# LGMOak/HighPerformanceComputing-LatticeBoltzmannMethod

Hardware: AMD Instinct MI355X
Metric: MLUPS (fp64) (higher is better)
Workload: dtype f64

## Files before the change

highperformancecomputing-latticeboltzmannmethod_amd/csrc/lbm_kernel_col.hpp:

```cpp
#pragma once
#include "lbm_kernels.hpp"

namespace lbmk {

__device__ __forceinline__ unsigned dpp_shr1(unsigned v) { return (unsigned)__builtin_amdgcn_mov_dpp((int)v, 0x138, 0xf, 0xf, true); }
__device__ __forceinline__ unsigned dpp_shl1(unsigned v) { return (unsigned)__builtin_amdgcn_mov_dpp((int)v, 0x130, 0xf, 0xf, true); }
__device__ __forceinline__ double from_left(double v) {
    const unsigned long long u = __builtin_bit_cast(unsigned long long, v);
    const unsigned lo = dpp_shr1((unsigned)u), hi = dpp_shr1((unsigned)(u >> 32));
    return __builtin_bit_cast(double, ((unsigned long long)hi << 32) | lo);
}
__device__ __forceinline__ double from_right(double v) {
    const unsigned long long u = __builtin_bit_cast(unsigned long long, v);
    const unsigned lo = dpp_shl1((unsigned)u), hi = dpp_shl1((unsigned)(u >> 32));
    return __builtin_bit_cast(double, ((unsigned long long)hi << 32) | lo);
}
__device__ __forceinline__ float from_left(float v) { return __builtin_bit_cast(float, dpp_shr1(__builtin_bit_cast(unsigned, v))); }
__device__ __forceinline__ float from_right(float v) { return __builtin_bit_cast(float, dpp_shl1(__builtin_bit_cast(unsigned, v))); }

template <int NW> constexpr int col_waves_per_simd() { return NW == 12 ? 6 : NW <= 8 ? (2 * NW) / 4 : NW / 4; }
template <typename T, int NW, int AR> constexpr int col_min_waves() {
    return (sizeof(T) == 4 && NW == 8 && AR == AR_CONTRACTED_TRT) ? 6 : col_waves_per_simd<NW>();
}

template <typename T, int R, int NW, int D, bool NT, int AR = AR_STRICT>
__global__ void __launch_bounds__(NW * 64, (col_min_waves<T, NW, AR>())) k_stepc_col(const KArgs<T> a, const K2Extra<T> e) {
    constexpr int H = R * NW, HW = D - 1, OW = 64 - 2 * HW, OH = H - 2 * HW, LW = 64 + 2;
    static_assert(D >= 2 && OH >= 1 && R >= 2, "(D <= GR on a strip: its ghost rows go GR deep — the host's business)");
    __shared__ T xbuf[2][NW][6][LW];
    const int lane = (int)threadIdx.x & 63;
    const int w = __builtin_amdgcn_readfirstlane((int)threadIdx.x >> 6);
    const int nbx = (a.nx + OW - 1) / OW, nby = (a.y_cnt + OH - 1) / OH + (a.y_cnt2 + OH - 1) / OH, nb = nbx * nby;
    int b = blockIdx.x;
    { const int per = (int)gridDim.x >> 3; b = (b & 7) * per + (b >> 3); }
    if (b >= nb) return;
    int by = b / nbx;
    const int bx = b - by * nbx;
    if (a.reverse) by = nby - 1 - by;
    int y_end;
    const int Yo = band_origin(a, by, OH, y_end);
    const int Xo = bx * OW;
    const int X0 = Xo - HW, Yr = Yo - HW;
    const int ry0 = w * R;
    const TileFrame<T> fr(a, e, Xo, Yo, y_end, OW, OH, HW);
    const int x = X0 + lane;
    auto run = [&]<bool LEAN>() {
        T g[R][Q];
        bool bad = false;
        const bool col_in = (x >= 0 && x < a.nx);
        unsigned sbits = 0;
        if (!LEAN && fr.near_solid && col_in) {
#pragma unroll
            for (int j = 0; j < R; ++j) {
                const int yg = a.y_start + Yr + ry0 + j;
                if (yg >= 0 && yg < a.ny_glob && solid_at(a, x, yg)) sbits |= 1u << j;
            }
        }
        LBM_PROF_IDS(b, NW, w);
        LBM_PROF(b, NW, w, 0);
        if (LEAN) {
            const unsigned ub = fr.src_off(a, Yr + ry0, X0), voff = (unsigned)lane * (unsigned)sizeof(T);
            auto load_all = [&]<int AUX>() {
#pragma unroll
                for (int j = 0; j < R; ++j) fr.template load<AUX>(g[j], voff, ub + (unsigned)j * fr.pitchB);
            };
            if (e.ntl) load_all.template operator()<2>(); else load_all.template operator()<0>();
#pragma unroll
            for (int j = 0; j < R; ++j) {
                bad |= any_unstable(g[j]);
                collide<T, AR>(g[j], a);
            }
        } else {
#pragma unroll
            for (int j = 0; j < R; ++j) {
                const int y = Yr + ry0 + j, yg = a.y_start + y;
                const bool row_in = (yg >= 0 && yg < a.ny_glob);
                if (!(row_in && col_in) || y > y_end + HW - 1) {
#pragma unroll
                    for (int i = 0; i < Q; ++i) g[j][i] = outside_value(e, row_in, col_in, i);
                } else {
                    const long c = (long)(y + GR) * a.pitch + a.xoff + x;
#pragma unroll
                    for (int i = 0; i < Q; ++i) g[j][i] = a.src[(long)i * a.plane + c - (long)cy(i) * a.pitch - cx(i)];
                    cell_update_as<T, AR, true>(a, g[j], x, yg, 0, (sbits >> j) & 1u, fr.near_solid, true, bad);
                }
            }
        }
        if (bad) atomicMin(a.unstable_t, *a.t_base + a.t);
        LBM_PROF(b, NW, w, 1);
        auto level = [&]<int L>() {
            T (*xb)[6][LW] = xbuf[L & 1];
            const int wb = w > 0 ? w - 1 : 0, wa = w + 1 < NW ? w + 1 : NW - 1;
            xb[w][0][1 + lane] = g[R - 1][2]; xb[w][1][1 + lane] = g[R - 1][5]; xb[w][2][1 + lane] = g[R - 1][6];
            xb[w][3][1 + lane] = g[0][4];     xb[w][4][1 + lane] = g[0][7];     xb[w][5][1 + lane] = g[0][8];
            __syncthreads();
            T p2 = xb[wb][0][1 + lane], p5 = xb[wb][1][lane], p6 = xb[wb][2][2 + lane];
            bool badl = false;
            const bool lane_ok = lane >= L - 1 && lane <= 64 - L;
#pragma unroll
            for (int j = 0; j < R; ++j) {
                const int ry = ry0 + j;
                const T n2 = g[j][2], n5 = g[j][5], n6 = g[j][6];
                if (ry >= L - 1 && ry <= H - L) {
                T f[Q];
                f[0] = g[j][0]; f[1] = from_left(g[j][1]); f[3] = from_right(g[j][3]);
                f[2] = p2; f[5] = p5; f[6] = p6;
                if (j < R - 1) { f[4] = g[j + 1][4]; f[7] = from_right(g[j + 1][7]); f[8] = from_left(g[j + 1][8]); }
                else { f[4] = xb[wa][3][1 + lane]; f[7] = xb[wa][4][2 + lane]; f[8] = xb[wa][5][lane]; }
                const bool valid = lane_ok;
                const int y = Yr + ry, yg = a.y_start + y;
                bool store = L == D && lane >= HW && lane < 64 - HW && ry >= HW && ry < H - HW;
                if (LEAN) {
                    badl |= unstable_if(f, valid);
                    collide<T, AR>(f, a);
                } else {
                    const bool row_in = (yg >= 0 && yg < a.ny_glob);
                    if (!(row_in && col_in)) {
#pragma unroll
                        for (int i = 0; i < Q; ++i) f[i] = outside_value(e, row_in, col_in, i);
                        store = false;
                    } else {
                        cell_update_as<T, AR, true>(a, f, x, yg, L - 1, (sbits >> j) & 1u, fr.near_solid, valid && y <= y_end + HW - L, badl);
                        store = store && y < y_end && !((sbits >> j) & 1u);
                    }
                }
                if (L < D) {
#pragma unroll
                    for (int i = 0; i < Q; ++i) g[j][i] = f[i];
                } else if (store) {
                    if (LEAN) fr.template store<NT>(f, (unsigned)lane * (unsigned)sizeof(T), fr.dst_off(a, y, X0));
                    else store_cell<NT>(a, f, x, y);
                }
                }
                if (j < R - 1) { p2 = n2; p5 = from_left(n5); p6 = from_right(n6); }
            }
            if (badl) atomicMin(a.unstable_t, *a.t_base + a.t + L - 1);
            LBM_PROF(b, NW, w, L);
        };
        [&]<int... Ls>(std::integer_sequence<int, Ls...>) { (level.template operator()<Ls + 2>(), ...); }(std::make_integer_sequence<int, D - 1>{});
    };
    if (fr.lean) run.template operator()<true>();
    else run.template operator()<false>();
}

}
```

highperformancecomputing-latticeboltzmannmethod_amd/csrc/lbm_kernels.hpp:

```cpp
#pragma once
#include <utility>
#include <hip/hip_runtime.h>

namespace lbmk {

constexpr int Q = 9;
constexpr int GR = 12;
constexpr int HR1 = 6;
__host__ __device__ constexpr int cx(int i) { constexpr int v[Q] = {0, 1, 0, -1, 0, 1, -1, -1, 1}; return v[i]; }
__host__ __device__ constexpr int cy(int i) { constexpr int v[Q] = {0, 0, 1, 0, -1, 1, 1, -1, -1}; return v[i]; }
__host__ __device__ constexpr int opp(int i) { constexpr int v[Q] = {0, 3, 4, 1, 2, 7, 8, 5, 6}; return v[i]; }
template <typename T> __host__ __device__ constexpr T wgt(int i) {
    return i == 0 ? T(4.0 / 9.0) : (i < 5 ? T(1.0 / 9.0) : T(1.0 / 36.0));
}

struct MaskView {
    const unsigned long long* bits = nullptr;
    const int* sat = nullptr;
    int y0 = 0, rows = 0, words = 0, nbx = 0, nby = 0;
};
__host__ __device__ inline bool mask_cell(const MaskView& m, int x, int yg) {
    const int r = yg - m.y0;
    if (r < 0 || r >= m.rows) return false;
    return (m.bits[(long)r * m.words + (x >> 6)] >> (x & 63)) & 1ull;
}
__host__ __device__ inline bool mask_box_any(const MaskView& m, int x0, int x1, int yg0, int yg1) {
    x0 = x0 < 0 ? 0 : x0;
    x1 = x1 > m.nbx * 8 - 1 ? m.nbx * 8 - 1 : x1;
    const int r0 = yg0 - m.y0 < 0 ? 0 : yg0 - m.y0, r1 = yg1 - m.y0 > m.rows - 1 ? m.rows - 1 : yg1 - m.y0;
    if (x0 > x1 || r0 > r1) return false;
    const int W = m.nbx + 1, c0 = x0 >> 3, c1 = (x1 >> 3) + 1, b0 = r0 >> 3, b1 = (r1 >> 3) + 1;
    return m.sat[b1 * W + c1] - m.sat[b0 * W + c1] - m.sat[b1 * W + c0] + m.sat[b0 * W + c0] > 0;
}

enum WallKind { WALL_NOSLIP = 0, WALL_FREESLIP = 1, WALL_MOVING = 2 };
__host__ __device__ constexpr int wall_pack(int south, int north) { return south | (north << 2); }
template <typename T> struct WallK { T s_add, s_sub, n_add, n_sub; };
template <typename T>
inline WallK<T> wall_ks(int south, double u_south, int north, double u_north) {
    WallK<T> k;
    k.s_add = south == WALL_MOVING ? (T)(u_south * (1.0 / 6.0)) : T(-0.0);
    k.s_sub = south == WALL_MOVING ? (T)(u_south * (1.0 / 6.0)) : T(0.0);
    k.n_add = north == WALL_MOVING ? (T)(u_north * (1.0 / 6.0)) : T(-0.0);
    k.n_sub = north == WALL_MOVING ? (T)(u_north * (1.0 / 6.0)) : T(0.0);
    return k;
}


template <typename T>
struct KArgs {
    const T* src;
    T* dst;
    long plane;
    int pitch;
    int xoff;
    int nx, ny_loc;
    int ny_glob;
    int y_start;
    int cyl_x, cyl_y;
    double cyl_r2;
    MaskView mv;
    T tau_inv;
    const T* u_row;
    int* unstable_t;
    int t;
    const int* t_base;
    int y_lo, y_cnt;
    int y_lo2, y_cnt2;
    int reverse;
    union { T les_tau; T trt_wm; };
    union { T les_tau2; T trt_wa; };
    union { T les_c; T trt_wb; };
    int walls;
    WallK<T> wk;
    const int* sched;
};

template <typename T>
__device__ __forceinline__ int row_of_block(const KArgs<T>& a) {
    const int by = (int)blockIdx.y;
    if (by >= a.y_cnt) return a.y_lo2 + (by - a.y_cnt);
    return a.y_lo + (a.reverse ? a.y_cnt - 1 - by : by);
}

template <typename T>
__device__ __forceinline__ int band_origin(const KArgs<T>& a, int by, int TY, int& y_end) {
    const int nb1 = (a.y_cnt + TY - 1) / TY;
    if (by >= nb1) { y_end = a.y_lo2 + a.y_cnt2; return a.y_lo2 + (by - nb1) * TY; }
    y_end = a.y_lo + a.y_cnt;
    return a.y_lo + by * TY;
}

__device__ __forceinline__ bool is_solid_cell(int x, int yg, int cyl_x, int cyl_y, double cyl_r2) {
    const double dx = (double)(x - cyl_x), dy = (double)(yg - cyl_y);
    return dx * dx + dy * dy <= cyl_r2;
}

template <typename A>
__device__ __forceinline__ bool solid_at(const A& a, int x, int yg) {
    return a.mv.bits ? mask_cell(a.mv, x, yg) : is_solid_cell(x, yg, a.cyl_x, a.cyl_y, a.cyl_r2);
}

template <typename T>
__device__ __forceinline__ bool tile_near_solid(const KArgs<T>& a, int X0, int Y0, int TX, int TY, int ring) {
    const int yg0 = a.y_start + Y0;
    if (a.mv.bits) return mask_box_any(a.mv, X0 - ring, X0 + TX - 1 + ring, yg0 - ring, yg0 + TY - 1 + ring);
    const int r = (int)sqrt(a.cyl_r2) + 1;
    return X0 - ring <= a.cyl_x + r && X0 + TX - 1 + ring >= a.cyl_x - r &&
           yg0 - ring <= a.cyl_y + r && yg0 + TY - 1 + ring >= a.cyl_y - r;
}

__host__ __device__ inline int inlet_sched_index(int t, int n, int mode) {
    const unsigned ut = (unsigned)t, un = (unsigned)n;
    return (int)(mode == 1 ? ut % un : (ut < un - 1u ? ut : un - 1u));
}
constexpr int INLET_SCHED_HEAD = 2;
template <typename T>
__device__ __forceinline__ T inlet_sched_at(const int* sched, int t) {
    return reinterpret_cast<const T*>(sched + INLET_SCHED_HEAD)[inlet_sched_index(t, sched[0], sched[1])];
}

template <typename T>
__host__ __device__ __forceinline__ void wall_rule(T (&f)[Q], bool bottom, bool top, int walls, const WallK<T>& k) {
    if (bottom) {
        const bool fs = (walls & 3) == WALL_FREESLIP;
        const T a = fs ? f[8] : f[7], b = fs ? f[7] : f[8];
        f[2] = f[4]; f[5] = a + k.s_add; f[6] = b - k.s_sub;
    }
    if (top) {
        const bool fs = ((walls >> 2) & 3) == WALL_FREESLIP;
        const T a = fs ? f[6] : f[5], b = fs ? f[5] : f[6];
        f[4] = f[2]; f[7] = a - k.n_sub; f[8] = b + k.n_add;
    }
}

template <typename T, typename U>
__device__ __forceinline__ void apply_bcs(T (&f)[Q], bool bottom, bool top, bool inlet, bool outlet, U&& inlet_u,
                                          int walls, const WallK<T>& wk, T& rho_bc, T& u_out) {
    wall_rule(f, bottom, top, walls, wk);
    if (inlet) {
        const T u_in = inlet_u();
        rho_bc = (f[0] + f[2] + f[4] + T(2.0) * (f[3] + f[6] + f[7])) / (T(1.0) - u_in);
        f[1] = f[3] + T(2.0 / 3.0) * rho_bc * u_in;
        f[5] = f[7] - T(0.5) * (f[2] - f[4]) + T(1.0 / 6.0) * rho_bc * u_in;
        f[8] = f[6] + T(0.5) * (f[2] - f[4]) + T(1.0 / 6.0) * rho_bc * u_in;
    }
    if (outlet) {
        const T rho_out = T(1.0);
        u_out = T(-1.0) + (f[0] + f[2] + f[4] + T(2.0) * (f[1] + f[5] + f[8])) / rho_out;
        f[3] = f[1] - T(2.0 / 3.0) * rho_out * u_out;
        f[6] = f[8] - T(0.5) * (f[2] - f[4]) - T(1.0 / 6.0) * rho_out * u_out;
        f[7] = f[5] + T(0.5) * (f[2] - f[4]) - T(1.0 / 6.0) * rho_out * u_out;
    }
}
template <typename T>
__device__ __forceinline__ void bcs_at(const KArgs<T>& a, T (&f)[Q], int x, int yg, int lvl) {
    T rho_bc, u_out;
    apply_bcs(f, yg == 0, yg == a.ny_glob - 1, x == 0, x == a.nx - 1, [&]() {
        T u = a.u_row[yg];
        if (a.sched) u = u * inlet_sched_at<T>(a.sched, *a.t_base + a.t + lvl);
        return u;
    }, a.walls, a.wk, rho_bc, u_out);
}

enum Arith { AR_STRICT = 0, AR_CONTRACTED = 1, AR_STRICT_LES = 2, AR_CONTRACTED_LES = 3, AR_STRICT_TRT = 4, AR_CONTRACTED_TRT = 5 };
constexpr bool ar_contracted(int ar) { return (ar & 1) != 0; }
constexpr bool ar_les(int ar) { return (ar & 2) != 0; }
constexpr bool ar_trt(int ar) { return (ar & 4) != 0; }
constexpr int ar_of(bool contracted, bool les, bool trt = false) { return (contracted ? 1 : 0) | (les ? 2 : 0) | (trt ? 4 : 0); }

__device__ __forceinline__ double fma_t(double a, double b, double c) { return __builtin_fma(a, b, c); }
__device__ __forceinline__ float fma_t(float a, float b, float c) { return __builtin_fmaf(a, b, c); }
__device__ __forceinline__ double recip_t(double d) {
    double r = __builtin_amdgcn_rcp(d);
    r = fma_t(fma_t(-d, r, 1.0), r, r);
    r = fma_t(fma_t(-d, r, 1.0), r, r);
    return r;
}
__device__ __forceinline__ float recip_t(float d) {
    float r = __builtin_amdgcn_rcpf(d);
    return fma_t(fma_t(-d, r, 1.0f), r, r);
}
__device__ __forceinline__ double sqrt_t(double v) { return __builtin_sqrt(v); }
__device__ __forceinline__ float sqrt_t(float v) { return __builtin_sqrtf(v); }
__device__ __forceinline__ double sqrt_c(double v) {
    v = __builtin_fmax(v, 1e-300);
    const double y = __builtin_amdgcn_rsq(v);
    const double s = v * y;
    return fma_t(s, fma_t(-s, 0.5 * y, 0.5), s);
}
__device__ __forceinline__ float sqrt_c(float v) { return __builtin_amdgcn_sqrtf(v); }

typedef unsigned lbm_u32x2 __attribute__((ext_vector_type(2)));
__device__ __forceinline__ __amdgpu_buffer_rsrc_t buf_desc(const void* base) {
    return __builtin_amdgcn_make_buffer_rsrc(const_cast<void*>(base), 0, 0xffffffff, 0x00020000);
}
template <typename T, int AUX = 0> __device__ __forceinline__ T buf_load(__amdgpu_buffer_rsrc_t r, unsigned voff, unsigned soff) {
    if constexpr (sizeof(T) == 8) return __builtin_bit_cast(T, __builtin_amdgcn_raw_buffer_load_b64(r, voff, soff, AUX));
    else return __builtin_bit_cast(T, __builtin_amdgcn_raw_buffer_load_b32(r, voff, soff, AUX));
}
template <bool NT> __device__ __forceinline__ void buf_store(double v, __amdgpu_buffer_rsrc_t r, unsigned voff, unsigned soff) {
    __builtin_amdgcn_raw_buffer_store_b64(__builtin_bit_cast(lbm_u32x2, v), r, voff, soff, NT ? 2 : 0);
}
template <bool NT> __device__ __forceinline__ void buf_store(float v, __amdgpu_buffer_rsrc_t r, unsigned voff, unsigned soff) {
    __builtin_amdgcn_raw_buffer_store_b32(__builtin_bit_cast(unsigned, v), r, voff, soff, NT ? 2 : 0);
}

__device__ __forceinline__ void strict_div2(double& a1, double& a2, double b) {
    double r = __builtin_amdgcn_rcp(b);
    double e = __builtin_fma(-b, r, 1.0);
    r = __builtin_fma(r, e, r);
    e = __builtin_fma(-b, r, 1.0);
    r = __builtin_fma(r, e, r);
    double q = a1 * r;
    a1 = __builtin_fma(__builtin_fma(-b, q, a1), r, q);
    q = a2 * r;
    a2 = __builtin_fma(__builtin_fma(-b, q, a2), r, q);
}
__device__ __forceinline__ void strict_div2(float& a1, float& a2, float b) { a1 /= b; a2 /= b; }
template <int UNUSED = 0>
__global__ void k_debug_strict_div2(const double* a1, const double* a2, const double* b, int n, double* q1, double* q2, double* r1, double* r2) {
    const int k = blockIdx.x * blockDim.x + threadIdx.x;
    if (k >= n) return;
    double x = a1[k], y = a2[k];
    strict_div2(x, y, b[k]);
    q1[k] = x; q2[k] = y;
    r1[k] = a1[k] / b[k]; r2[k] = a2[k] / b[k];
}

template <typename T>
__device__ __forceinline__ T les_tau_inv_strict(const T (&f)[Q], T rho, T ux, T uy, T tau, T tau2, T c) {
    const T sxx = ((((f[1] + f[3]) + f[5]) + f[6]) + f[7]) + f[8];
    const T syy = ((((f[2] + f[4]) + f[5]) + f[6]) + f[7]) + f[8];
    const T sxy = ((f[5] - f[6]) + f[7]) - f[8];
    const T pxx = (sxx - rho * (ux * ux)) - rho * T(1.0 / 3.0);
    const T pyy = (syy - rho * (uy * uy)) - rho * T(1.0 / 3.0);
    const T pxy = sxy - rho * (ux * uy);
    const T qn = sqrt_t((pxx * pxx + pyy * pyy) + T(2.0) * (pxy * pxy));
    const T tau_eff = T(0.5) * (tau + sqrt_t(tau2 + c * (qn / rho)));
    return T(1.0) / tau_eff;
}

template <typename T, int AR = AR_STRICT>
__device__ __forceinline__ void bgk_collide(T (&f)[Q], T tau_inv, T les_tau = T(0), T les_tau2 = T(0), T les_c = T(0)) {
    T rho = T(0), ux = T(0), uy = T(0);
    if constexpr (ar_contracted(AR)) {
        const T a13 = f[1] + f[3], a24 = f[2] + f[4], a57 = f[5] + f[7], a68 = f[6] + f[8];
        const T d13 = f[1] - f[3], d24 = f[2] - f[4], d57 = f[5] - f[7], d68 = f[6] - f[8];
        rho = ((f[0] + a13) + (a24 + a57)) + a68;
        ux = (d13 + d57) - d68;
        uy = (d24 + d57) + d68;
        const T rinv = recip_t(rho);
        const T inv3 = rinv * T(3.0);
        const T vx = ux * inv3, vy = uy * inv3;
        if constexpr (ar_les(AR)) {
            const T sxx = (a13 + a57) + a68, syy = (a24 + a57) + a68, sxy = a57 - a68;
            const T jxr = ux * rinv;
            const T third = rho * T(-1.0 / 3.0);
            const T pxx = fma_t(-jxr, ux, sxx + third), pyy = fma_t(-uy * rinv, uy, syy + third), pxy = fma_t(-jxr, uy, sxy);
            const T qn = sqrt_c(fma_t(pxx, pxx, fma_t(pyy, pyy, T(2.0) * (pxy * pxy))));
            tau_inv = T(2.0) * recip_t(les_tau + sqrt_c(fma_t(les_c, qn * rinv, les_tau2)));
        }
        const T base = fma_t(T(-1.0 / 6.0), fma_t(vx, vx, vy * vy), T(1.0));
        const T wr0 = wgt<T>(0) * rho, wr1 = wgt<T>(1) * rho, wr5 = wgt<T>(5) * rho;
        if constexpr (ar_trt(AR)) {
            const T wa = les_tau2, wb = les_c;
            f[0] = fma_t(tau_inv, fma_t(wr0, base, -f[0]), f[0]);
            auto pair = [&](int i, int ib, T cv, T wr) {
                const T ri = fma_t(wr, fma_t(cv, fma_t(cv, T(0.5), T(1.0)), base), -f[i]);
                const T rb = fma_t(wr, fma_t(cv, fma_t(cv, T(0.5), T(-1.0)), base), -f[ib]);
                f[i] = fma_t(wa, ri, fma_t(wb, rb, f[i]));
                f[ib] = fma_t(wa, rb, fma_t(wb, ri, f[ib]));
            };
            auto then = [&](int i, int ib, int j, int jb) { asm volatile("" : "+v"(f[i]), "+v"(f[ib]), "+v"(f[j]), "+v"(f[jb])); };
            pair(5, 7, vx + vy, wr5);
            then(5, 7, 8, 6);
            pair(8, 6, vx - vy, wr5);
            then(8, 6, 1, 3);
            pair(1, 3, vx, wr1);
            then(1, 3, 2, 4);
            pair(2, 4, vy, wr1);
            return;
        }
#pragma unroll
        for (int i = 0; i < Q; ++i) {
            T cv;
            if (cx(i) == 0 && cy(i) == 0) cv = T(0);
            else if (cy(i) == 0) cv = T(cx(i)) * vx;
            else if (cx(i) == 0) cv = T(cy(i)) * vy;
            else cv = T(cx(i)) * vx + T(cy(i)) * vy;
            const T t = (i == 0) ? base : fma_t(cv, fma_t(cv, T(0.5), T(1.0)), base);
            const T wr = i == 0 ? wr0 : (i < 5 ? wr1 : wr5);
            f[i] = fma_t(tau_inv, fma_t(wr, t, -f[i]), f[i]);
        }
        return;
    }
#pragma unroll
    for (int i = 0; i < Q; ++i) {
        rho += f[i];
        if (cx(i) != 0) ux += T(cx(i)) * f[i];
        if (cy(i) != 0) uy += T(cy(i)) * f[i];
    }
    strict_div2(ux, uy, rho);
    if constexpr (ar_les(AR)) tau_inv = les_tau_inv_strict(f, rho, ux, uy, les_tau, les_tau2, les_c);
    const T usq = ux * ux + uy * uy;
    const T c15 = T(1.5) * usq;
    const T wr0 = wgt<T>(0) * rho, wr1 = wgt<T>(1) * rho, wr5 = wgt<T>(5) * rho;
    auto relax = [&](T& fi, T wr, T bracket) {
        const T feq = wr * bracket;
        fi = fi - tau_inv * (fi - feq);
    };
    relax(f[0], wr0, (T(1.0) + T(0.0)) - c15);
    auto pair = [&](int i, int ib, T cu, T wr) {
        const T t3 = T(3.0) * cu, t45 = (T(4.5) * cu) * cu;
        if constexpr (ar_trt(AR)) {
            const T feq = wr * (((T(1.0) + t3) + t45) - c15), feqb = wr * (((T(1.0) - t3) + t45) - c15);
            const T np = T(0.5) * ((f[i] + f[ib]) - (feq + feqb));
            const T nm = T(0.5) * ((f[i] - f[ib]) - (feq - feqb));
            const T wpn = tau_inv * np, wmn = les_tau * nm;
            f[i] = (f[i] - wpn) - wmn;
            f[ib] = (f[ib] - wpn) + wmn;
            return;
        }
        relax(f[i], wr, ((T(1.0) + t3) + t45) - c15);
        relax(f[ib], wr, ((T(1.0) - t3) + t45) - c15);
    };
    pair(1, 3, ux, wr1);
    pair(2, 4, uy, wr1);
    pair(5, 7, ux + uy, wr5);
    pair(8, 6, ux - uy, wr5);
}

template <typename T, int AR>
__device__ __forceinline__ void collide(T (&f)[Q], const KArgs<T>& a) {
    static_assert(!(ar_les(AR) && ar_trt(AR)), "TRT and LES exclude each other");
    if constexpr (ar_trt(AR)) bgk_collide<T, AR>(f, a.tau_inv, a.trt_wm, a.trt_wa, a.trt_wb);
    else if constexpr (ar_les(AR)) bgk_collide<T, AR>(f, T(0), a.les_tau, a.les_tau2, a.les_c);
    else bgk_collide<T, AR>(f, a.tau_inv);
}

__device__ __forceinline__ unsigned exp_word(double v) { return (unsigned)(__builtin_bit_cast(unsigned long long, v) >> 32); }
__device__ __forceinline__ unsigned exp_word(float v) { return __builtin_bit_cast(unsigned, v); }
template <typename T>
__device__ __forceinline__ bool any_unstable(const T (&f)[Q]) {
    unsigned o = 0;
#pragma unroll
    for (int i = 0; i < Q; ++i) o |= exp_word(f[i]);
    bool bad = false;
    if (o & 0x40000000u) {
#pragma unroll
        for (int i = 0; i < Q; ++i) bad |= !(fabs(f[i]) <= T(1e5));
    }
    return bad;
}
template <typename T>
__device__ __forceinline__ bool unstable_if(const T (&f)[Q], bool valid) {
    unsigned o = 0;
#pragma unroll
    for (int i = 0; i < Q; ++i) o |= exp_word(f[i]);
    o = valid ? o : 0u;
    bool bad = false;
    if (o & 0x40000000u) {
#pragma unroll
        for (int i = 0; i < Q; ++i) bad |= !(fabs(f[i]) <= T(1e5));
        bad = bad && valid;
    }
    return bad;
}

enum StepMode { MODE_STEP = 0, MODE_COLLIDE_ONLY = 1, MODE_STREAM_ONLY = 2 };

template <typename T, int MODE, bool NT = false, int AR = AR_STRICT>
__global__ void __launch_bounds__(256) k_step_site(const KArgs<T> a) {
    const int x = blockIdx.x * 256 + threadIdx.x;
    const int y = row_of_block(a);
    if (x >= a.nx) return;
    const int yg = a.y_start + y;
    const long c = (long)(y + GR) * a.pitch + a.xoff + x;
    T f[Q];
#pragma unroll
    for (int i = 0; i < Q; ++i) {
        const long off = (MODE == MODE_COLLIDE_ONLY) ? 0 : (long)cy(i) * a.pitch + cx(i);
        f[i] = a.src[(long)i * a.plane + c - off];
    }
    const bool solid = solid_at(a, x, yg);
    if (MODE != MODE_COLLIDE_ONLY && !solid) bcs_at(a, f, x, yg, 0);
    if (MODE == MODE_STEP) {
        if (any_unstable(f)) atomicMin(a.unstable_t, *a.t_base + a.t);
    }
    if (MODE == MODE_STREAM_ONLY) {
        if (solid) {
            T r[Q];
#pragma unroll
            for (int i = 0; i < Q; ++i) r[i] = f[opp(i)];
#pragma unroll
            for (int i = 0; i < Q; ++i) f[i] = r[i];
        }
    } else {
        if (solid) return;
        collide<T, AR>(f, a);
    }
#pragma unroll
    for (int i = 0; i < Q; ++i) {
        T* p = a.dst + (long)i * a.plane + c;
        if (NT) __builtin_nontemporal_store(f[i], p);
        else *p = f[i];
    }
}


template <typename T> struct K2Extra {
    const T* feq_in;
    int small;
    int xcd;
    int nt;
    int ntl;
};


template <typename T, int AR, bool BRANCH_FREE = false>
__device__ __forceinline__ void cell_update_as(const KArgs<T>& a, T (&f)[Q], int x, int yg, int lvl, bool solid, bool near_solid,
                                               bool count, bool& bad) {
    if (!solid) bcs_at(a, f, x, yg, lvl);
    if (BRANCH_FREE) bad |= unstable_if(f, count);
    else if (count) bad |= any_unstable(f);
    collide<T, AR>(f, a);
    if (near_solid) {
#pragma unroll
        for (int i = 0; i < Q; ++i) f[i] = solid ? wgt<T>(i) : f[i];
    }
}
template <typename T, int AR>
__device__ __forceinline__ void cell_update(const KArgs<T>& a, T (&f)[Q], int x, int yg, int lvl, bool near_solid, bool count, bool& bad) {
    bool solid = false;
    if (near_solid) solid = solid_at(a, x, yg);
    cell_update_as<T, AR>(a, f, x, yg, lvl, solid, near_solid, count, bad);
}
template <typename T, int AR>
__device__ __forceinline__ bool cell_update_last(const KArgs<T>& a, T (&f)[Q], int x, int yg, int lvl, bool near_solid, bool& bad) {
    const bool solid = near_solid && solid_at(a, x, yg);
    if (!solid) bcs_at(a, f, x, yg, lvl);
    bad |= any_unstable(f);
    if (solid) return false;
    collide<T, AR>(f, a);
    return true;
}

template <typename T>
__device__ __forceinline__ T outside_value(const K2Extra<T>& e, bool row_in, bool col_in, int i) {
    return (row_in && !col_in) ? T(0) : e.feq_in[i];
}
template <bool NT, typename T>
__device__ __forceinline__ void store_cell(const KArgs<T>& a, const T (&f)[Q], int x, int y) {
    T* base = a.dst + ((long)(y + GR) * a.pitch + a.xoff + x);
#pragma unroll
    for (int i = 0; i < Q; ++i) {
        if (NT) __builtin_nontemporal_store(f[i], base + (long)i * a.plane); else base[(long)i * a.plane] = f[i];
    }
}
template <typename T>
__device__ __forceinline__ void store_cell(const KArgs<T>& a, const T (&f)[Q], int x, int y, bool nt) {
    if (nt) store_cell<true>(a, f, x, y); else store_cell<false>(a, f, x, y);
}

template <typename T>
struct TileFrame {
    int X0, Y0;
    int y_end;
    bool near_solid;
    bool lean;
    unsigned pitchB, planeB, KB;
    __amdgpu_buffer_rsrc_t rsrc, rdst;

    __device__ __forceinline__ TileFrame(const KArgs<T>& a, const K2Extra<T>& e, int X0_, int Y0_, int y_end_, int OW, int OH, int HW)
        : X0(X0_), Y0(Y0_), y_end(y_end_) {
        near_solid = tile_near_solid(a, X0, Y0, OW, OH, HW);
        const int yg0 = a.y_start + Y0;
        lean = !near_solid && X0 >= HW + 1 && X0 + OW + HW <= a.nx - 1 && yg0 >= HW + 1 && yg0 + OH + HW <= a.ny_glob - 1 &&
               Y0 + OH <= y_end && e.small;
        pitchB = (unsigned)a.pitch * (unsigned)sizeof(T);
        planeB = (unsigned)a.plane * (unsigned)sizeof(T);
        KB = pitchB + (unsigned)sizeof(T);
        rsrc = buf_desc(reinterpret_cast<const char*>(a.src) - KB);
        rdst = buf_desc(a.dst);
    }
    __device__ __forceinline__ unsigned src_off(const KArgs<T>& a, int y, int x) const {
        return (unsigned)(y + GR) * pitchB + (unsigned)(a.xoff + x) * (unsigned)sizeof(T) + KB;
    }
    __device__ __forceinline__ unsigned dst_off(const KArgs<T>& a, int y, int x) const {
        return (unsigned)(y + GR) * pitchB + (unsigned)(a.xoff + x) * (unsigned)sizeof(T);
    }
    __device__ __forceinline__ unsigned at(int row, int col) const { return (unsigned)row * pitchB + (unsigned)col * (unsigned)sizeof(T); }
    template <int AUX = 0>
    __device__ __forceinline__ void load(T (&f)[Q], unsigned voff, unsigned soff) const {
#pragma unroll
        for (int i = 0; i < Q; ++i)
            f[i] = buf_load<T, AUX>(rsrc, voff, soff + (unsigned)i * planeB - (unsigned)cy(i) * pitchB - (unsigned)(cx(i) * (int)sizeof(T)));
    }
    template <bool NT>
    __device__ __forceinline__ void store(const T (&f)[Q], unsigned voff, unsigned soff) const {
#pragma unroll
        for (int i = 0; i < Q; ++i) buf_store<NT>(f[i], rdst, voff, soff + (unsigned)i * planeB);
    }
    __device__ __forceinline__ void store(const T (&f)[Q], unsigned voff, unsigned soff, bool nt) const {
        if (nt) store<true>(f, voff, soff); else store<false>(f, voff, soff);
    }
};

template <typename T>
__device__ __forceinline__ TileFrame<T> tile_frame(const KArgs<T>& a, const K2Extra<T>& e, int TX, int TY, int HW) {
    int bx = blockIdx.x, by = blockIdx.y;
    if (e.xcd) {
        const int nb = gridDim.x * gridDim.y;
        int b = by * gridDim.x + bx;
        if (nb % 8 == 0) b = (b % 8) * (nb / 8) + b / 8;
        by = b / gridDim.x; bx = b - by * gridDim.x;
    }
    if (a.reverse) by = (int)gridDim.y - 1 - by;
    int y_end;
    const int Y0 = band_origin(a, by, TY, y_end);
    return TileFrame<T>(a, e, bx * TX, Y0, y_end, TX, TY, HW);
}

template <typename T, int TY, int NTH, int AR = AR_STRICT>
__global__ void __launch_bounds__(NTH) k_step2_tile(const KArgs<T> a, const K2Extra<T> e) {
    constexpr int TX = 64, RW = TX + 2, RH = TY + 2, LP = RW + 2;
    __shared__ T lds[Q][RH][LP];
    const TileFrame<T> fr = tile_frame(a, e, TX, TY, 1);
    const int X0 = fr.X0, Y0 = fr.Y0, y_end = fr.y_end;
    bool bad = false;
    for (int r = threadIdx.x; r < RW * RH; r += NTH) {
        const int ry = r / RW, rx = r - ry * RW;
        const int x = X0 + rx - 1, y = Y0 + ry - 1;
        if (y > y_end) continue;
        const int yg = a.y_start + y;
        const bool row_in = (yg >= 0 && yg < a.ny_glob), col_in = (x >= 0 && x < a.nx);
        T f[Q];
        if (!(row_in && col_in)) {
#pragma unroll
            for (int i = 0; i < Q; ++i) f[i] = outside_value(e, row_in, col_in, i);
        } else {
            const long c = (long)(y + GR) * a.pitch + a.xoff + x;
#pragma unroll
            for (int i = 0; i < Q; ++i) f[i] = a.src[(long)i * a.plane + c - (long)cy(i) * a.pitch - cx(i)];
            cell_update<T, AR>(a, f, x, yg, 0, fr.near_solid, true, bad);
        }
#pragma unroll
        for (int i = 0; i < Q; ++i) lds[i][ry][rx] = f[i];
    }
    if (bad) atomicMin(a.unstable_t, *a.t_base + a.t);
    __syncthreads();
    bad = false;
    for (int o = threadIdx.x; o < TX * TY; o += NTH) {
        const int ly = o / TX, lx = o - ly * TX;
        const int x = X0 + lx, y = Y0 + ly;
        if (y >= y_end || x >= a.nx) continue;
        T f[Q];
#pragma unroll
        for (int i = 0; i < Q; ++i) f[i] = lds[i][ly + 1 - cy(i)][lx + 1 - cx(i)];
        if (cell_update_last<T, AR>(a, f, x, a.y_start + y, 1, fr.near_solid, bad)) store_cell(a, f, x, y, e.nt != 0);
    }
    if (bad) atomicMin(a.unstable_t, *a.t_base + a.t + 1);
}

template <typename T, int TY, int NTH, int D, int AR>
__device__ __forceinline__ void step_tile(const KArgs<T>& a, const K2Extra<T>& e) {
    constexpr int TX = 64, HW = D - 1, R1W = TX + 2 * HW, R1H = TY + 2 * HW, LP = R1W;
    static_assert((R1W - 2) * (R1H - 2) <= 2 * NTH, "two cells per thread at most in the in-place levels");
    __shared__ T lds[Q][R1H][LP];
    const TileFrame<T> fr = tile_frame(a, e, TX, TY, HW);
    const int X0 = fr.X0, Y0 = fr.Y0, y_end = fr.y_end;
    auto run = [&]<bool LEAN>() {
        bool bad = false;
#pragma unroll
        for (int r = threadIdx.x; r < R1W * R1H; r += NTH) {
            const int ry = r / R1W, rx = r - ry * R1W;
            T f[Q];
            if (LEAN) {
                fr.load(f, fr.at(ry, rx), fr.src_off(a, Y0 - HW, X0 - HW));
                bad |= any_unstable(f);
                collide<T, AR>(f, a);
            } else {
                const int x = X0 + rx - HW, y = Y0 + ry - HW;
                const int yg = a.y_start + y;
                const bool row_in = (yg >= 0 && yg < a.ny_glob), col_in = (x >= 0 && x < a.nx);
                if (!(row_in && col_in) || y > y_end + HW - 1) {
#pragma unroll
                    for (int i = 0; i < Q; ++i) f[i] = outside_value(e, row_in, col_in, i);
                } else {
                    const long c = (long)(y + GR) * a.pitch + a.xoff + x;
#pragma unroll
                    for (int i = 0; i < Q; ++i) f[i] = a.src[(long)i * a.plane + c - (long)cy(i) * a.pitch - cx(i)];
                    cell_update<T, AR>(a, f, x, yg, 0, fr.near_solid, true, bad);
                }
            }
#pragma unroll
            for (int i = 0; i < Q; ++i) lds[i][ry][rx] = f[i];
        }
        if (bad) atomicMin(a.unstable_t, *a.t_base + a.t);
        __syncthreads();
        auto in_place = [&]<int L>() {
            constexpr int O = L - 1, RW = R1W - 2 * O, RH = R1H - 2 * O;
            T g[2][Q];
            int cell[2];
#pragma unroll
            for (int k = 0; k < 2; ++k) {
                const int r = (int)threadIdx.x + k * NTH;
                cell[k] = (r < RW * RH) ? r : -1;
                if (cell[k] >= 0) {
                    const int ry = r / RW + O, rx = r - (r / RW) * RW + O;
#pragma unroll
                    for (int i = 0; i < Q; ++i) g[k][i] = lds[i][ry - cy(i)][rx - cx(i)];
                }
            }
            __syncthreads();
            bool badl = false;
#pragma unroll
            for (int k = 0; k < 2; ++k) {
                if (cell[k] < 0) continue;
                const int r = cell[k];
                const int ry = r / RW + O, rx = r - (r / RW) * RW + O;
                const int x = X0 + rx - HW, y = Y0 + ry - HW;
                const int yg = a.y_start + y;
                const bool row_in = (yg >= 0 && yg < a.ny_glob), col_in = (x >= 0 && x < a.nx);
                T f[Q];
                if (!LEAN && !(row_in && col_in)) {
#pragma unroll
                    for (int i = 0; i < Q; ++i) f[i] = outside_value(e, row_in, col_in, i);
                } else {
#pragma unroll
                    for (int i = 0; i < Q; ++i) f[i] = g[k][i];
                    if (LEAN) {
                        badl |= any_unstable(f);
                        collide<T, AR>(f, a);
                    } else cell_update<T, AR>(a, f, x, yg, L - 1, fr.near_solid, y <= y_end + HW - L, badl);
                }
#pragma unroll
                for (int i = 0; i < Q; ++i) lds[i][ry][rx] = f[i];
            }
            if (badl) atomicMin(a.unstable_t, *a.t_base + a.t + L - 1);
            __syncthreads();
        };
        [&]<int... Ls>(std::integer_sequence<int, Ls...>) { (in_place.template operator()<Ls + 2>(), ...); }(std::make_integer_sequence<int, D - 2>{});
        bad = false;
        for (int o = threadIdx.x; o < TX * TY; o += NTH) {
            const int ly = o / TX, lx = o - ly * TX;
            const int x = X0 + lx, y = Y0 + ly;
            if (!LEAN && (y >= y_end || x >= a.nx)) continue;
            T f[Q];
#pragma unroll
            for (int i = 0; i < Q; ++i) f[i] = lds[i][ly + HW - cy(i)][lx + HW - cx(i)];
            if (LEAN) {
                bad |= any_unstable(f);
                collide<T, AR>(f, a);
                fr.store(f, fr.at(ly, lx), fr.dst_off(a, Y0, X0), e.nt != 0);
            } else if (cell_update_last<T, AR>(a, f, x, a.y_start + y, D - 1, fr.near_solid, bad)) store_cell(a, f, x, y, e.nt != 0);
        }
        if (bad) atomicMin(a.unstable_t, *a.t_base + a.t + D - 1);
    };
    if (fr.lean) run.template operator()<true>();
    else run.template operator()<false>();
}
template <typename T, int TY, int NTH, int AR = AR_STRICT>
__global__ void __launch_bounds__(NTH, (2 * NTH / 256)) k_step3_tile(const KArgs<T> a, const K2Extra<T> e) { step_tile<T, TY, NTH, 3, AR>(a, e); }
template <typename T, int TY, int NTH, int AR = AR_STRICT>
__global__ void __launch_bounds__(NTH, (2 * NTH / 256)) k_step4_tile(const KArgs<T> a, const K2Extra<T> e) { step_tile<T, TY, NTH, 4, AR>(a, e); }

#ifdef LBM_COL_PROF
constexpr int PROF_SLOTS = 96;
__device__ unsigned long long* lbm_prof_buf;
__device__ __forceinline__ void prof_mark(int blk, int nw, int w, int slot) {
    asm volatile("" ::: "memory");
    if (((int)threadIdx.x & 63) == 0 && slot < PROF_SLOTS) {
        unsigned long long t;
        asm volatile("s_memrealtime %0\n\ts_waitcnt lgkmcnt(0)" : "=s"(t) :: "memory");
        lbm_prof_buf[((size_t)blk * nw + w) * PROF_SLOTS + slot] = t;
    }
    asm volatile("" ::: "memory");
}
__device__ __forceinline__ void prof_ids(int blk, int nw, int w) {
    if (((int)threadIdx.x & 63) == 0) {
        const unsigned hw = __builtin_amdgcn_s_getreg(4 | (0 << 6) | (31 << 11)), xcc = __builtin_amdgcn_s_getreg(20 | (0 << 6) | (31 << 11));
        unsigned long long rt;
        asm volatile("s_memrealtime %0\n\ts_waitcnt lgkmcnt(0)" : "=s"(rt) :: "memory");
        lbm_prof_buf[((size_t)blk * nw + w) * PROF_SLOTS + PROF_SLOTS - 1] = ((unsigned long long)xcc << 32) | hw;
        lbm_prof_buf[((size_t)blk * nw + w) * PROF_SLOTS + PROF_SLOTS - 2] = rt;
    }
}
#define LBM_PROF(blk, nw, w, slot) prof_mark(blk, nw, w, slot)
#define LBM_PROF_IDS(blk, nw, w) prof_ids(blk, nw, w)
#else
#define LBM_PROF(blk, nw, w, slot) do {} while (0)
#define LBM_PROF_IDS(blk, nw, w) do {} while (0)
#endif

template <typename T, int TX, int TY, int D>
constexpr int deep_waves_per_simd() {
    const int lds = (int)sizeof(T) * Q * (TX + 2 * (D - 1)) * (TY + 2 * (D - 1)), waves = TX * TY / 64;
    int blocks = 160 * 1024 / lds;
    if (blocks * waves > 32) blocks = 32 / waves;
    return (blocks * waves) / 4 > 0 ? (blocks * waves) / 4 : 1;
}
template <typename T, int TX, int TY, int D, int AR = AR_STRICT>
__global__ void __launch_bounds__(TX * TY, (deep_waves_per_simd<T, TX, TY, D>())) k_stepd_tile(const KArgs<T> a, const K2Extra<T> e) {
    constexpr int NTH = TX * TY, HW = D - 1, R1W = TX + 2 * HW, R1H = TY + 2 * HW, LP = R1W;
    static_assert(D >= 3 && (NTH == 1024 || NTH == 512 || NTH == 256), "one tile cell per thread at the last level");
    static_assert((TX & (TX - 1)) == 0, "cell_xy splits an index with a mask");
    static_assert((size_t)Q * R1H * LP * sizeof(T) <= 160 * 1024, "level-1 region must fit the CU's LDS");
    __shared__ T lds[Q][R1H][LP];
    auto cell_xy = [&]<int O>(int r, int& ry, int& rx) {
        constexpr int RH = R1H - 2 * O, HALO = HW - O, NC = RH * TX;
        if (HALO == 0 || r < NC) { ry = O + r / TX; rx = HW + (r & (TX - 1)); }
        else {
            const int h = r - NC, q = h / (2 * HALO), c = h - q * (2 * HALO);
            ry = O + q;
            rx = c < HALO ? O + c : HW + TX + (c - HALO);
        }
    };
    const TileFrame<T> fr = tile_frame(a, e, TX, TY, HW);
    const int X0 = fr.X0, Y0 = fr.Y0, y_end = fr.y_end;
    auto run = [&]<bool LEAN>() {
        bool bad = false;
        [[maybe_unused]] const int pb = (int)(blockIdx.y * gridDim.x + blockIdx.x), pw = (int)threadIdx.x >> 6;
        LBM_PROF_IDS(pb, NTH / 64, pw);
        LBM_PROF(pb, NTH / 64, pw, 0);
#pragma unroll
        for (int r = threadIdx.x; r < R1W * R1H; r += NTH) {
            int ry, rx;
            cell_xy.template operator()<0>(r, ry, rx);
            T f[Q];
            if (LEAN) {
                fr.load(f, fr.at(ry, rx), fr.src_off(a, Y0 - HW, X0 - HW));
                bad |= any_unstable(f);
// ... 384 lines not shown
```

Measured before the change: 155,900.

## Restructure non-lean column path: batch loads, mask words, shared inlet velocities

```diff
diff --git a/highperformancecomputing-latticeboltzmannmethod_amd/csrc/lbm_kernel_col.hpp b/highperformancecomputing-latticeboltzmannmethod_amd/csrc/lbm_kernel_col.hpp
--- a/highperformancecomputing-latticeboltzmannmethod_amd/csrc/lbm_kernel_col.hpp
+++ b/highperformancecomputing-latticeboltzmannmethod_amd/csrc/lbm_kernel_col.hpp
@@ -28,6 +28,7 @@
     constexpr int H = R * NW, HW = D - 1, OW = 64 - 2 * HW, OH = H - 2 * HW, LW = 64 + 2;
     static_assert(D >= 2 && OH >= 1 && R >= 2, "(D <= GR on a strip: its ghost rows go GR deep — the host's business)");
     __shared__ T xbuf[2][NW][6][LW];
+    __shared__ T u_sh[NW][R];
     const int lane = (int)threadIdx.x & 63;
     const int w = __builtin_amdgcn_readfirstlane((int)threadIdx.x >> 6);
     const int nbx = (a.nx + OW - 1) / OW, nby = (a.y_cnt + OH - 1) / OH + (a.y_cnt2 + OH - 1) / OH, nb = nbx * nby;
@@ -49,12 +50,31 @@
         bool bad = false;
         const bool col_in = (x >= 0 && x < a.nx);
         unsigned sbits = 0;
-        if (!LEAN && fr.near_solid && col_in) {
+        unsigned long long mw[R];
+        unsigned rin = 0, rld = 0;
+        const bool masked = !LEAN && fr.near_solid && a.mv.bits != nullptr;
+        if (!LEAN) {
 #pragma unroll
             for (int j = 0; j < R; ++j) {
-                const int yg = a.y_start + Yr + ry0 + j;
-                if (yg >= 0 && yg < a.ny_glob && solid_at(a, x, yg)) sbits |= 1u << j;
+                const int y = Yr + ry0 + j, yg = a.y_start + y;
+                mw[j] = 0;
+                if (yg >= 0 && yg < a.ny_glob) { rin |= 1u << j; if (y <= y_end + HW - 1) rld |= 1u << j; }
             }
+            if (fr.near_solid && col_in) {
+#pragma unroll
+                for (int j = 0; j < R; ++j) {
+                    const int yg = a.y_start + Yr + ry0 + j;
+                    if ((rin >> j) & 1u) {
+                        if (masked) mw[j] = mask_word(a.mv, x, yg);
+                        else if (is_solid_cell(x, yg, a.cyl_x, a.cyl_y, a.cyl_r2)) sbits |= 1u << j;
+                    }
+                }
+            }
+            if (bx == 0 && lane < R) {
+                const int yg = a.y_start + Yr + ry0 + lane;
+                u_sh[w][lane] = (yg >= 0 && yg < a.ny_glob) ? a.u_row[yg] : T(0);
+            }
+            __builtin_amdgcn_wave_barrier();
         }
         LBM_PROF_IDS(b, NW, w);
         LBM_PROF(b, NW, w, 0);
@@ -73,16 +93,42 @@
         } else {
 #pragma unroll
             for (int j = 0; j < R; ++j) {
-                const int y = Yr + ry0 + j, yg = a.y_start + y;
-                const bool row_in = (yg >= 0 && yg < a.ny_glob);
-                if (!(row_in && col_in) || y > y_end + HW - 1) {
+                const bool row_in = (rin >> j) & 1u;
+                if (!((rld >> j) & 1u)) {
+                    const T* fq = e.feq_in;
+                    asm volatile("" : "+v"(fq));
 #pragma unroll
-                    for (int i = 0; i < Q; ++i) g[j][i] = outside_value(e, row_in, col_in, i);
-                } else {
-                    const long c = (long)(y + GR) * a.pitch + a.xoff + x;
+                    for (int i = 0; i < Q; ++i) g[j][i] = T(0);
+                    if (!(row_in && !col_in)) {
 #pragma unroll
-                    for (int i = 0; i < Q; ++i) g[j][i] = a.src[(long)i * a.plane + c - (long)cy(i) * a.pitch - cx(i)];
-                    cell_update_as<T, AR, true>(a, g[j], x, yg, 0, (sbits >> j) & 1u, fr.near_solid, true, bad);
+                        for (int i = 0; i < Q; ++i) g[j][i] = fq[i];
+                    }
+                }
+            }
+#pragma unroll
+            for (int j = 0; j < R; ++j) {
+                const int y = Yr + ry0 + j;
+                if ((rld >> j) & 1u) {
+#pragma unroll
+                    for (int i = 0; i < Q; ++i) g[j][i] = T(0);
+                    if (col_in) {
+                        const long c = (long)(y + GR) * a.pitch + a.xoff + x;
+#pragma unroll
+                        for (int i = 0; i < Q; ++i) g[j][i] = a.src[(long)i * a.plane + c - (long)cy(i) * a.pitch - cx(i)];
+                    }
+                }
+            }
+            if (masked) {
+#pragma unroll
+                for (int j = 0; j < R; ++j) sbits |= (unsigned)((mw[j] >> (x & 63)) & 1ull) << j;
+            }
+#pragma unroll
+            for (int j = 0; j < R; ++j) {
+                const int yg = a.y_start + Yr + ry0 + j;
+                if ((rld >> j) & 1u) {
+                    cell_update_with<T, AR, true>(a, g[j], x, yg, 0, (sbits >> j) & 1u, fr.near_solid, col_in, bad, [&]() { return u_sh[w][j]; });
+#pragma unroll
+                    for (int i = 0; i < Q; ++i) g[j][i] = col_in ? g[j][i] : T(0);
                 }
             }
         }
@@ -101,28 +147,24 @@
             for (int j = 0; j < R; ++j) {
                 const int ry = ry0 + j;
                 const T n2 = g[j][2], n5 = g[j][5], n6 = g[j][6];
-                if (ry >= L - 1 && ry <= H - L) {
+                const int y = Yr + ry, yg = a.y_start + y;
+                if (ry >= L - 1 && ry <= H - L && (LEAN || ((rin >> j) & 1u))) {
                 T f[Q];
                 f[0] = g[j][0]; f[1] = from_left(g[j][1]); f[3] = from_right(g[j][3]);
                 f[2] = p2; f[5] = p5; f[6] = p6;
                 if (j < R - 1) { f[4] = g[j + 1][4]; f[7] = from_right(g[j + 1][7]); f[8] = from_left(g[j + 1][8]); }
                 else { f[4] = xb[wa][3][1 + lane]; f[7] = xb[wa][4][2 + lane]; f[8] = xb[wa][5][lane]; }
                 const bool valid = lane_ok;
-                const int y = Yr + ry, yg = a.y_start + y;
                 bool store = L == D && lane >= HW && lane < 64 - HW && ry >= HW && ry < H - HW;
                 if (LEAN) {
                     badl |= unstable_if(f, valid);
                     collide<T, AR>(f, a);
                 } else {
-                    const bool row_in = (yg >= 0 && yg < a.ny_glob);
-                    if (!(row_in && col_in)) {
+                    cell_update_with<T, AR, true>(a, f, x, yg, L - 1, (sbits >> j) & 1u, fr.near_solid,
+                                                  valid && col_in && y <= y_end + HW - L, badl, [&]() { return u_sh[w][j]; });
 #pragma unroll
-                        for (int i = 0; i < Q; ++i) f[i] = outside_value(e, row_in, col_in, i);
-                        store = false;
-                    } else {
-                        cell_update_as<T, AR, true>(a, f, x, yg, L - 1, (sbits >> j) & 1u, fr.near_solid, valid && y <= y_end + HW - L, badl);
-                        store = store && y < y_end && !((sbits >> j) & 1u);
-                    }
+                    for (int i = 0; i < Q; ++i) f[i] = col_in ? f[i] : T(0);
+                    store = store && col_in && y < y_end && !((sbits >> j) & 1u);
                 }
                 if (L < D) {
 #pragma unroll
diff --git a/highperformancecomputing-latticeboltzmannmethod_amd/csrc/lbm_kernels.hpp b/highperformancecomputing-latticeboltzmannmethod_amd/csrc/lbm_kernels.hpp
--- a/highperformancecomputing-latticeboltzmannmethod_amd/csrc/lbm_kernels.hpp
+++ b/highperformancecomputing-latticeboltzmannmethod_amd/csrc/lbm_kernels.hpp
@@ -23,6 +23,10 @@
     const int r = yg - m.y0;
     if (r < 0 || r >= m.rows) return false;
     return (m.bits[(long)r * m.words + (x >> 6)] >> (x & 63)) & 1ull;
+}
+__device__ __forceinline__ unsigned long long mask_word(const MaskView& m, int x, int yg) {
+    const int r = yg - m.y0;
+    return (r < 0 || r >= m.rows) ? 0ull : m.bits[(long)r * m.words + (x >> 6)];
 }
 __host__ __device__ inline bool mask_box_any(const MaskView& m, int x0, int x1, int yg0, int yg1) {
     x0 = x0 < 0 ? 0 : x0;
@@ -153,14 +157,18 @@
         f[7] = f[5] + T(0.5) * (f[2] - f[4]) - T(1.0 / 6.0) * rho_out * u_out;
     }
 }
-template <typename T>
-__device__ __forceinline__ void bcs_at(const KArgs<T>& a, T (&f)[Q], int x, int yg, int lvl) {
+template <typename T, typename U>
+__device__ __forceinline__ void bcs_at_with(const KArgs<T>& a, T (&f)[Q], int x, int yg, int lvl, U&& row_u) {
     T rho_bc, u_out;
     apply_bcs(f, yg == 0, yg == a.ny_glob - 1, x == 0, x == a.nx - 1, [&]() {
-        T u = a.u_row[yg];
+        T u = row_u();
         if (a.sched) u = u * inlet_sched_at<T>(a.sched, *a.t_base + a.t + lvl);
         return u;
     }, a.walls, a.wk, rho_bc, u_out);
+}
+template <typename T>
+__device__ __forceinline__ void bcs_at(const KArgs<T>& a, T (&f)[Q], int x, int yg, int lvl) {
+    bcs_at_with(a, f, x, yg, lvl, [&]() { return a.u_row[yg]; });
 }
 
 enum Arith { AR_STRICT = 0, AR_CONTRACTED = 1, AR_STRICT_LES = 2, AR_CONTRACTED_LES = 3, AR_STRICT_TRT = 4, AR_CONTRACTED_TRT = 5 };
@@ -418,10 +426,10 @@
 };
 
 
-template <typename T, int AR, bool BRANCH_FREE = false>
-__device__ __forceinline__ void cell_update_as(const KArgs<T>& a, T (&f)[Q], int x, int yg, int lvl, bool solid, bool near_solid,
-                                               bool count, bool& bad) {
-    if (!solid) bcs_at(a, f, x, yg, lvl);
+template <typename T, int AR, bool BRANCH_FREE = false, typename U>
+__device__ __forceinline__ void cell_update_with(const KArgs<T>& a, T (&f)[Q], int x, int yg, int lvl, bool solid, bool near_solid,
+                                                 bool count, bool& bad, U&& row_u) {
+    if (!solid) bcs_at_with(a, f, x, yg, lvl, row_u);
     if (BRANCH_FREE) bad |= unstable_if(f, count);
     else if (count) bad |= any_unstable(f);
     collide<T, AR>(f, a);
@@ -429,6 +437,11 @@
 #pragma unroll
         for (int i = 0; i < Q; ++i) f[i] = solid ? wgt<T>(i) : f[i];
     }
+}
+template <typename T, int AR, bool BRANCH_FREE = false>
+__device__ __forceinline__ void cell_update_as(const KArgs<T>& a, T (&f)[Q], int x, int yg, int lvl, bool solid, bool near_solid,
+                                               bool count, bool& bad) {
+    cell_update_with<T, AR, BRANCH_FREE>(a, f, x, yg, lvl, solid, near_solid, count, bad, [&]() { return a.u_row[yg]; });
 }
 template <typename T, int AR>
 __device__ __forceinline__ void cell_update(const KArgs<T>& a, T (&f)[Q], int x, int yg, int lvl, bool near_solid, bool count, bool& bad) {
```

New measurement: 163,900 (median of 6 runs). 5.2% higher.
